# L0SG/grouped-ssd-pytorch

Measured on AMD Instinct MI355X. Metric: 512x512 4-phase CT img/s (fwd+loss), higher is better.
Workload: dtype f32; 1 GPU; gssdpp (BASELINE configs[2], GSSD++: self-attention + SA-base + 1 DCN layer x 4 deformable groups, dcn_cat_sab) fwd + MultiBoxLoss, train-mode BN, batch 32, [B,12,300,300] slices; batch_per_gpu=32, global_batch=32

## Files before the change

grouped-ssd-pytorch_amd/gssd/csrc/conv_patch_x6.hip:

```cpp
#include "common.h"
#include "kernel_util.h"
#include <cstdlib>

namespace {

__device__ __attribute__((aligned(16))) float g_zero_px6[4] = {0.f, 0.f, 0.f, 0.f};

constexpr int TH = 8, TW = 16, PW = TW + 2, PHT = TH + 2, NPATCH = PHT * PW;
constexpr int NPAD = 192, CK = 32, BN = 128, NTHR = 256, NSTG = 3;
constexpr int PLANE = NPAD * CK;
constexpr int WPLANE = BN * CK;
constexpr int WSTAGE = 2 * WPLANE;
constexpr int LDS_BYTES = (2 * PLANE + NSTG * WSTAGE) * 2;
constexpr int NLD = NPAD * (CK / 4) / NTHR;

__device__ __forceinline__ int swz_a(int col) { return (col >> 1) & 2; }

struct PatchX6Params {
    const float* in;
    const u16* wp;
    const float* bias;
    float* out;
    int B, H, W, C, in_stride, Cout, out_stride, out_ch_off, tiles_y, tiles_x, relu;
};

__global__ __launch_bounds__(NTHR, 2) void conv_patch_x6_kernel(const PatchX6Params p) {
    extern __shared__ __attribute__((aligned(16))) u16 smem[];
    u16* const planes = smem;
    u16* const wring = smem + 2 * PLANE;
    const int tid = threadIdx.x, lane = tid & 63;
    const int wave = __builtin_amdgcn_readfirstlane(tid >> 6);
    const int r = lane & 15, kq = lane >> 4;
    const int ntiles = p.B * p.tiles_y * p.tiles_x;
    const int per = (ntiles + 7) >> 3;
    const int tile = (int)(blockIdx.x & 7) * per + (int)(blockIdx.x >> 3);
    if ((int)(blockIdx.x >> 3) >= per || tile >= ntiles) return;
    const int tpi = p.tiles_y * p.tiles_x;
    const int b = tile / tpi, trem = tile - b * tpi;
    const int y0 = (trem / p.tiles_x) * TH, x0 = (trem % p.tiles_x) * TW;
    const int nchunks = p.C / CK, nsteps = nchunks * 9;

    const int su = tid & 7, pp0 = tid >> 3;
    const float* src[NLD];
    int wr[NLD];
#pragma unroll
    for (int it = 0; it < NLD; ++it) {
        const int pp = pp0 + 32 * it;
        const int py = pp / PW, px = pp - py * PW;
        const int iy = y0 - 1 + py, ix = x0 - 1 + px;
        const bool ok = pp < NPATCH && (unsigned)iy < (unsigned)p.H && (unsigned)ix < (unsigned)p.W;
        src[it] = ok ? p.in + ((size_t)(b * p.H + iy) * p.W + ix) * p.in_stride + 4 * su : nullptr;
        wr[it] = pp * CK + (((su >> 1) ^ swz_a(px)) << 3) + 4 * (su & 1);
    }
    f32x4 pre[NLD];
    auto load_chunk = [&](int cc) {
#pragma unroll
        for (int it = 0; it < NLD; ++it) pre[it] = src[it] ? *reinterpret_cast<const f32x4*>(src[it] + cc * CK) : f32x4{0.f, 0.f, 0.f, 0.f};
    };
    auto write_planes = [&]() {
#pragma unroll
        for (int it = 0; it < NLD; ++it) {
            unsigned h0, l0, h1, l1;
            split2_pair(pre[it][0], pre[it][1], h0, l0);
            split2_pair(pre[it][2], pre[it][3], h1, l1);
            *reinterpret_cast<u32x2*>(planes + wr[it]) = u32x2{h0, h1};
            *reinterpret_cast<u32x2*>(planes + PLANE + wr[it]) = u32x2{l0, l1};
        }
    };
    auto dma_stage = [&](int s) {
        const u16* g = p.wp + (size_t)s * WSTAGE + lane * 8;
        u16* d = wring + (s % NSTG) * WSTAGE;
#pragma unroll
        for (int q = 0; q < 4; ++q) {
            const int piece = 4 * q + wave;
            dma16(g + piece * 512, d + piece * 512);
        }
    };

    f32x4 acc[TH][2], acx[TH][2];
#pragma unroll
    for (int i = 0; i < TH; ++i)
#pragma unroll
        for (int j = 0; j < 2; ++j) acc[i][j] = acx[i][j] = f32x4{0.f, 0.f, 0.f, 0.f};

    load_chunk(0);
    dma_stage(0);
    dma_stage(1);
    write_planes();
    if (nchunks > 1) load_chunk(1);

    const int boff = (32 * wave + r) * CK + ((kq ^ swz64(r)) << 3);
    for (int s = 0; s < nsteps; ++s) {
        const int cc = s / 9, tap = s - cc * 9;
        const int dy = tap / 3, dx = tap - dy * 3;
        if (s == nsteps - 1) asm volatile("s_waitcnt vmcnt(0) lgkmcnt(0)\n\ts_barrier" ::: "memory");
        else if (tap == 1 && cc + 1 < nchunks) asm volatile("s_waitcnt vmcnt(10) lgkmcnt(0)\n\ts_barrier" ::: "memory");
        else asm volatile("s_waitcnt vmcnt(4) lgkmcnt(0)\n\ts_barrier" ::: "memory");
        if (s + 2 < nsteps) dma_stage(s + 2);
        if (tap == 0 && s > 0 && cc + 1 < nchunks) load_chunk(cc + 1);
        const u16* wst = wring + (s % NSTG) * WSTAGE;
        f16x8 bh[2], bl[2];
#pragma unroll
        for (int j = 0; j < 2; ++j) {
            bh[j] = *reinterpret_cast<const f16x8*>(wst + boff + j * 16 * CK);
            bl[j] = *reinterpret_cast<const f16x8*>(wst + WPLANE + boff + j * 16 * CK);
        }
        const int col = r + dx;
        const int aoff = col * CK + ((kq ^ swz_a(col)) << 3);
#pragma unroll
        for (int i = 0; i < TH; ++i) {
            const u16* ap = planes + (i + dy) * (PW * CK) + aoff;
            const f16x8 ah = *reinterpret_cast<const f16x8*>(ap);
            const f16x8 al = *reinterpret_cast<const f16x8*>(ap + PLANE);
            acx[i][0] = __builtin_amdgcn_mfma_f32_16x16x32_f16(bl[0], ah, acx[i][0], 0, 0, 0);
            acx[i][1] = __builtin_amdgcn_mfma_f32_16x16x32_f16(bl[1], ah, acx[i][1], 0, 0, 0);
            acc[i][0] = __builtin_amdgcn_mfma_f32_16x16x32_f16(bh[0], ah, acc[i][0], 0, 0, 0);
            acc[i][1] = __builtin_amdgcn_mfma_f32_16x16x32_f16(bh[1], ah, acc[i][1], 0, 0, 0);
            acx[i][0] = __builtin_amdgcn_mfma_f32_16x16x32_f16(bh[0], al, acx[i][0], 0, 0, 0);
            acx[i][1] = __builtin_amdgcn_mfma_f32_16x16x32_f16(bh[1], al, acx[i][1], 0, 0, 0);
        }
        if (tap == 8 && cc + 1 < nchunks) {
            asm volatile("s_waitcnt lgkmcnt(0)\n\ts_barrier" ::: "memory");
            write_planes();
        }
    }

    const int x = x0 + r;
#pragma unroll
    for (int j = 0; j < 2; ++j) {
        const int n0 = 32 * wave + 16 * j + 4 * kq;
        if (n0 >= p.Cout) continue;
        f32x4 bv = {0.f, 0.f, 0.f, 0.f};
        if (p.bias) bv = *reinterpret_cast<const f32x4*>(p.bias + n0);
#pragma unroll
        for (int i = 0; i < TH; ++i) {
            const int y = y0 + i;
            if (y >= p.H || x >= p.W) continue;
            f32x4 v;
#pragma unroll
            for (int e = 0; e < 4; ++e) {
                v[e] = __builtin_fmaf(acx[i][j][e], 1.f / 2048.f, acc[i][j][e]) + bv[e];
                if (p.relu) v[e] = fmaxf(v[e], 0.f);
            }
            *reinterpret_cast<f32x4*>(p.out + ((size_t)(b * p.H + y) * p.W + x) * p.out_stride + p.out_ch_off + n0) = v;
        }
    }
}

__global__ void conv_patch_x6_pack_kernel(const float* __restrict__ w, u16* __restrict__ wp, int Cout, int C, int row_stride, long long total) {
    for (long long i = blockIdx.x * (long long)blockDim.x + threadIdx.x; i < total; i += (long long)gridDim.x * blockDim.x) {
        const int e = (int)(i & 7), slot = (int)((i >> 3) & 3), row = (int)((i >> 5) & (BN - 1));
        const long long s = i >> 12;
        const int cc = (int)(s / 9), tap = (int)(s - 9 * (long long)cc);
        const int c = cc * CK + ((slot ^ swz64(row)) << 3) + e;
        const float v = row < Cout ? w[(size_t)row * row_stride + (size_t)tap * C + c] : 0.f;
        const _Float16 h = (_Float16)v;
        wp[s * WSTAGE + (i & (WPLANE - 1))] = __builtin_bit_cast(u16, h);
        wp[s * WSTAGE + WPLANE + (i & (WPLANE - 1))] = __builtin_bit_cast(u16, (_Float16)((v - (float)h) * 2048.f));
    }
}

bool px6_enabled() {
    static const bool on = !gssd_env_off("GSSD_PATCH_X6") && gssd_x6_f16_enabled();
    return on;
}

}

extern "C" long long gssd_conv_patch_x6_weight_elems(int Cout, int C) {
    if (Cout <= 0 || Cout > BN || Cout % 4 != 0 || C <= 0 || C % CK != 0) return -1;
    return 2ll * BN * 9 * C;
}

extern "C" int gssd_conv_patch_x6_pack_weight(const float* w_packed, void* out, int Cout, int C, int row_stride, gssd_stream_t stream) {
    GSSD_CHECK_ARG(w_packed && out && row_stride >= 9 * C && gssd_conv_patch_x6_weight_elems(Cout, C) > 0);
    const long long total = (long long)BN * 9 * C;
    hipLaunchKernelGGL(conv_patch_x6_pack_kernel, dim3((int)((total + 255) / 256 > 16384 ? 16384 : (total + 255) / 256)), dim3(256), 0, as_stream(stream),
                       w_packed, reinterpret_cast<u16*>(out), Cout, C, row_stride, total);
    GSSD_CHECK_LAUNCH();
    return GSSD_OK;
}

extern "C" int gssd_conv_patch_x6_takes(const gssd_conv_desc* dp) {
    if (!dp || !px6_enabled()) return 0;
    const gssd_conv_desc& d = *dp;
    if (!d.wgt_patch || !(d.flags & GSSD_CONV_F16_OK) || (d.flags & ~(GSSD_CONV_F16_OK | GSSD_CONV_OUT_F32))) return 0;
    if (d.groups != 1 || d.KH != 3 || d.KW != 3 || d.stride != 1 || d.pad != 1 || d.dil != 1 || d.Ho != d.H || d.Wo != d.W) return 0;
    if (gssd_conv_patch_x6_weight_elems(d.Cout, d.cin_g) <= 0) return 0;
    if (d.out_mode != GSSD_OUT_NHWC || d.m_per_image || d.split_k > 1 || d.in_scale || d.stats || d.alpha || d.gate || d.resid || d.out2) return 0;
    if (d.in_stride % 4 || d.in_ch_off % 4 || d.out_stride % 4 || d.out_ch_off % 4) return 0;
    if (((uintptr_t)d.in % 16) || ((uintptr_t)d.out % 16) || ((uintptr_t)d.wgt_patch % 16) || (d.bias && ((uintptr_t)d.bias % 16))) return 0;
    if ((long long)d.B * d.H * d.W * d.in_stride >= (1ll << 31)) return 0;
    return 1;
}

int gssd_try_conv_patch_x6(const gssd_conv_desc& d, gssd_conv_ctx& c) {
    if (!gssd_conv_patch_x6_takes(&d)) return 1;
    if (c.name) return gssd_name_kernel(c, "conv_patch_x6<%d>", BN);
    PatchX6Params p;
    p.in = d.in + d.in_ch_off;
    p.wp = reinterpret_cast<const u16*>(d.wgt_patch);
    p.bias = d.bias;
    p.out = d.out;
    p.B = d.B;
    p.H = d.H;
    p.W = d.W;
    p.C = d.cin_g;
    p.in_stride = d.in_stride;
    p.Cout = d.Cout;
    p.out_stride = d.out_stride;
    p.out_ch_off = d.out_ch_off;
    p.tiles_y = (d.H + TH - 1) / TH;
    p.tiles_x = (d.W + TW - 1) / TW;
    p.relu = d.relu;
    static unsigned attr_mask = 0;
    auto kern = conv_patch_x6_kernel;
    if (const int rc = gssd_max_dynamic_lds(&attr_mask, kern, LDS_BYTES)) return rc;
    const int ntiles = p.B * p.tiles_y * p.tiles_x;
    const int per = (ntiles + 7) / 8;
    hipLaunchKernelGGL(kern, dim3(per * 8), dim3(NTHR), LDS_BYTES, c.stream, p);
    GSSD_CHECK_LAUNCH();
    return GSSD_OK;
}
```

Before: 4926 img/s.

## Add flattened strip tiling to x6 patch conv with padded-width row runs

Adds an alternative tiling for the split-f16 3x3 conv kernel. Each block now covers a contiguous strip of 16-pixel runs over a padded-width flattened image instead of an 8x16 tile, so halo columns are shared along rows and fewer tiles are wasted on partial widths. The run count (4, 6 or 8) is chosen per shape from the CU count and can be overridden by an environment variable. Fewer accumulator rows with small runs change register pressure, and the padded columns add some wasted MMA work. Out-of-bounds loads now read a zero buffer instead of using a select.

```diff
diff --git a/grouped-ssd-pytorch_amd/gssd/csrc/conv_patch_x6.hip b/grouped-ssd-pytorch_amd/gssd/csrc/conv_patch_x6.hip
--- a/grouped-ssd-pytorch_amd/gssd/csrc/conv_patch_x6.hip
+++ b/grouped-ssd-pytorch_amd/gssd/csrc/conv_patch_x6.hip
@@ -7,37 +7,45 @@
 __device__ __attribute__((aligned(16))) float g_zero_px6[4] = {0.f, 0.f, 0.f, 0.f};
 
 constexpr int TH = 8, TW = 16, PW = TW + 2, PHT = TH + 2, NPATCH = PHT * PW;
-constexpr int NPAD = 192, CK = 32, BN = 128, NTHR = 256, NSTG = 3;
-constexpr int PLANE = NPAD * CK;
+constexpr int CK = 32, BN = 128, NTHR = 256, NSTG = 3;
 constexpr int WPLANE = BN * CK;
 constexpr int WSTAGE = 2 * WPLANE;
-constexpr int LDS_BYTES = (2 * PLANE + NSTG * WSTAGE) * 2;
-constexpr int NLD = NPAD * (CK / 4) / NTHR;
-
-__device__ __forceinline__ int swz_a(int col) { return (col >> 1) & 2; }
+constexpr int lds_bytes(int npad) { return (2 * npad * CK + NSTG * WSTAGE) * 2; }
+constexpr int strip_pixels(int runs, int wp) { return 16 * runs + 2 * wp + 2; }
+
+__device__ __forceinline__ int swz_a(int px) { return (px >> 1) & 2; }
 
 struct PatchX6Params {
     const float* in;
     const u16* wp;
     const float* bias;
     float* out;
-    int B, H, W, C, in_stride, Cout, out_stride, out_ch_off, tiles_y, tiles_x, relu;
+    int B, H, W, C, in_stride, Cout, out_stride, out_ch_off, relu;
+    int tiles_y, tiles_x;
+    int Wp, strips;
 };
 
+template <int R, int NPAD>
 __global__ __launch_bounds__(NTHR, 2) void conv_patch_x6_kernel(const PatchX6Params p) {
+    constexpr bool STRIP = R > 0;
+    constexpr int ROWS = STRIP ? R : TH;
+    constexpr int PLANE = NPAD * CK;
+    constexpr int NLD = NPAD * (CK / 4) / NTHR;
+    static_assert(NPAD % 32 == 0 && NPAD >= NPATCH, "whole staging passes that hold the 8 x 16 form's patch");
     extern __shared__ __attribute__((aligned(16))) u16 smem[];
     u16* const planes = smem;
     u16* const wring = smem + 2 * PLANE;
     const int tid = threadIdx.x, lane = tid & 63;
     const int wave = __builtin_amdgcn_readfirstlane(tid >> 6);
     const int r = lane & 15, kq = lane >> 4;
-    const int ntiles = p.B * p.tiles_y * p.tiles_x;
+    const int tpi = STRIP ? p.strips : p.tiles_y * p.tiles_x;
+    const int ntiles = p.B * tpi;
     const int per = (ntiles + 7) >> 3;
     const int tile = (int)(blockIdx.x & 7) * per + (int)(blockIdx.x >> 3);
     if ((int)(blockIdx.x >> 3) >= per || tile >= ntiles) return;
-    const int tpi = p.tiles_y * p.tiles_x;
     const int b = tile / tpi, trem = tile - b * tpi;
-    const int y0 = (trem / p.tiles_x) * TH, x0 = (trem % p.tiles_x) * TW;
+    const int y0 = STRIP ? 0 : (trem / p.tiles_x) * TH, x0 = STRIP ? 0 : (trem % p.tiles_x) * TW;
+    const int q0 = trem * (16 * ROWS);
     const int nchunks = p.C / CK, nsteps = nchunks * 9;
 
     const int su = tid & 7, pp0 = tid >> 3;
@@ -46,16 +54,25 @@
 #pragma unroll
     for (int it = 0; it < NLD; ++it) {
         const int pp = pp0 + 32 * it;
-        const int py = pp / PW, px = pp - py * PW;
-        const int iy = y0 - 1 + py, ix = x0 - 1 + px;
-        const bool ok = pp < NPATCH && (unsigned)iy < (unsigned)p.H && (unsigned)ix < (unsigned)p.W;
+        int iy, ix, key;
+        bool ok;
+        if constexpr (STRIP) {
+            const int py = (q0 + pp) / p.Wp, px = (q0 + pp) - py * p.Wp;
+            iy = py - 1, ix = px - 1, key = pp;
+            ok = pp < strip_pixels(R, p.Wp);
+        } else {
+            const int py = pp / PW, px = pp - py * PW;
+            iy = y0 - 1 + py, ix = x0 - 1 + px, key = px;
+            ok = pp < NPATCH;
+        }
+        ok = ok && (unsigned)iy < (unsigned)p.H && (unsigned)ix < (unsigned)p.W;
         src[it] = ok ? p.in + ((size_t)(b * p.H + iy) * p.W + ix) * p.in_stride + 4 * su : nullptr;
-        wr[it] = pp * CK + (((su >> 1) ^ swz_a(px)) << 3) + 4 * (su & 1);
+        wr[it] = pp * CK + (((su >> 1) ^ swz_a(key)) << 3) + 4 * (su & 1);
     }
     f32x4 pre[NLD];
     auto load_chunk = [&](int cc) {
 #pragma unroll
-        for (int it = 0; it < NLD; ++it) pre[it] = src[it] ? *reinterpret_cast<const f32x4*>(src[it] + cc * CK) : f32x4{0.f, 0.f, 0.f, 0.f};
+        for (int it = 0; it < NLD; ++it) pre[it] = *reinterpret_cast<const f32x4*>(src[it] ? src[it] + cc * CK : g_zero_px6);
     };
     auto write_planes = [&]() {
 #pragma unroll
@@ -77,9 +94,9 @@
         }
     };
 
-    f32x4 acc[TH][2], acx[TH][2];
-#pragma unroll
-    for (int i = 0; i < TH; ++i)
+    f32x4 acc[ROWS][2], acx[ROWS][2];
+#pragma unroll
+    for (int i = 0; i < ROWS; ++i)
 #pragma unroll
         for (int j = 0; j < 2; ++j) acc[i][j] = acx[i][j] = f32x4{0.f, 0.f, 0.f, 0.f};
 
@@ -94,7 +111,7 @@
         const int cc = s / 9, tap = s - cc * 9;
         const int dy = tap / 3, dx = tap - dy * 3;
         if (s == nsteps - 1) asm volatile("s_waitcnt vmcnt(0) lgkmcnt(0)\n\ts_barrier" ::: "memory");
-        else if (tap == 1 && cc + 1 < nchunks) asm volatile("s_waitcnt vmcnt(10) lgkmcnt(0)\n\ts_barrier" ::: "memory");
+        else if (tap == 1 && cc + 1 < nchunks) asm volatile("s_waitcnt vmcnt(%0) lgkmcnt(0)\n\ts_barrier" ::"n"(4 + NLD) : "memory");
         else asm volatile("s_waitcnt vmcnt(4) lgkmcnt(0)\n\ts_barrier" ::: "memory");
         if (s + 2 < nsteps) dma_stage(s + 2);
         if (tap == 0 && s > 0 && cc + 1 < nchunks) load_chunk(cc + 1);
@@ -105,11 +122,13 @@
             bh[j] = *reinterpret_cast<const f16x8*>(wst + boff + j * 16 * CK);
             bl[j] = *reinterpret_cast<const f16x8*>(wst + WPLANE + boff + j * 16 * CK);
         }
+        constexpr int ASTEP = STRIP ? 16 : PW;
         const int col = r + dx;
-        const int aoff = col * CK + ((kq ^ swz_a(col)) << 3);
-#pragma unroll
-        for (int i = 0; i < TH; ++i) {
-            const u16* ap = planes + (i + dy) * (PW * CK) + aoff;
+        const int a0 = STRIP ? dy * p.Wp + col : dy * PW + col;
+        const int aoff = a0 * CK + ((kq ^ swz_a(STRIP ? a0 : col)) << 3);
+#pragma unroll
+        for (int i = 0; i < ROWS; ++i) {
+            const u16* ap = planes + i * (ASTEP * CK) + aoff;
             const f16x8 ah = *reinterpret_cast<const f16x8*>(ap);
             const f16x8 al = *reinterpret_cast<const f16x8*>(ap + PLANE);
             acx[i][0] = __builtin_amdgcn_mfma_f32_16x16x32_f16(bl[0], ah, acx[i][0], 0, 0, 0);
@@ -125,7 +144,6 @@
         }
     }
 
-    const int x = x0 + r;
 #pragma unroll
     for (int j = 0; j < 2; ++j) {
         const int n0 = 32 * wave + 16 * j + 4 * kq;
@@ -133,8 +151,9 @@
         f32x4 bv = {0.f, 0.f, 0.f, 0.f};
         if (p.bias) bv = *reinterpret_cast<const f32x4*>(p.bias + n0);
 #pragma unroll
-        for (int i = 0; i < TH; ++i) {
-            const int y = y0 + i;
+        for (int i = 0; i < ROWS; ++i) {
+            const int o = q0 + 16 * i + r;
+            const int y = STRIP ? o / p.Wp : y0 + i, x = STRIP ? o - y * p.Wp : x0 + r;
             if (y >= p.H || x >= p.W) continue;
             f32x4 v;
 #pragma unroll
@@ -163,6 +182,29 @@
 bool px6_enabled() {
     static const bool on = !gssd_env_off("GSSD_PATCH_X6") && gssd_x6_f16_enabled();
     return on;
+}
+
+constexpr int strip_npad(int runs) { return runs == 8 ? 224 : 192; }
+
+int pick_strip_runs(int B, int H, int Wp) {
+    static const int env = [] {
+        const char* e = getenv("GSSD_PATCH_X6_STRIPS");
+        return e && e[0] ? atoi(e) : -1;
+    }();
+    if (env == 0) return 0;
+    const auto fits = [&](int runs) { return strip_pixels(runs, Wp) <= strip_npad(runs); };
+    if ((env == 4 || env == 6 || env == 8) && fits(env)) return env;
+    int dev = 0, ncu = 256;
+    (void)hipGetDevice(&dev);
+    if (hipDeviceGetAttribute(&ncu, hipDeviceAttributeMultiprocessorCount, dev) != hipSuccess || ncu <= 0) ncu = 256;
+    const int nruns = (H * Wp + 15) / 16;
+    int best = 0;
+    for (const int runs : {4, 6, 8}) {
+        if (!fits(runs)) continue;
+        best = runs;
+        if ((long long)B * ((nruns + runs - 1) / runs) <= 2ll * ncu) break;
+    }
+    return best;
 }
 
 }
@@ -213,12 +255,22 @@
     p.tiles_y = (d.H + TH - 1) / TH;
     p.tiles_x = (d.W + TW - 1) / TW;
     p.relu = d.relu;
-    static unsigned attr_mask = 0;
-    auto kern = conv_patch_x6_kernel;
-    if (const int rc = gssd_max_dynamic_lds(&attr_mask, kern, LDS_BYTES)) return rc;
-    const int ntiles = p.B * p.tiles_y * p.tiles_x;
-    const int per = (ntiles + 7) / 8;
-    hipLaunchKernelGGL(kern, dim3(per * 8), dim3(NTHR), LDS_BYTES, c.stream, p);
-    GSSD_CHECK_LAUNCH();
-    return GSSD_OK;
-}
+    p.Wp = (d.W + 2 + 7) / 8 * 8;
+    const int runs = pick_strip_runs(d.B, d.H, p.Wp);
+    p.strips = runs ? ((d.H * p.Wp + 15) / 16 + runs - 1) / runs : 0;
+    const int ntiles = runs ? p.B * p.strips : p.B * p.tiles_y * p.tiles_x;
+    const int blocks = (ntiles + 7) / 8 * 8;
+    static unsigned attr_mask[4] = {0, 0, 0, 0};
+    auto launch = [&](auto kern, unsigned* mask, int lds) -> int {
+        if (const int rc = gssd_max_dynamic_lds(mask, kern, lds)) return rc;
+        hipLaunchKernelGGL(kern, dim3(blocks), dim3(NTHR), lds, c.stream, p);
+        GSSD_CHECK_LAUNCH();
+        return GSSD_OK;
+    };
+    switch (runs) {
+        case 4: return launch(conv_patch_x6_kernel<4, strip_npad(4)>, &attr_mask[1], lds_bytes(strip_npad(4)));
+        case 6: return launch(conv_patch_x6_kernel<6, strip_npad(6)>, &attr_mask[2], lds_bytes(strip_npad(6)));
+        case 8: return launch(conv_patch_x6_kernel<8, strip_npad(8)>, &attr_mask[3], lds_bytes(strip_npad(8)));
+        default: return launch(conv_patch_x6_kernel<0, 192>, &attr_mask[0], lds_bytes(192));
+    }
+}
```

Result: no change. 4955 img/s (median of 6 runs) (+0.6%).
